# facebookresearch/holo_diffusion

Measured on AMD Instinct MI355X. Metric: denoise-steps/sec + rendered-rays/sec, 64^3x32 grid @400^2 render, higher is better.
Workload: dtype f32

## Files before the change

holo_diffusion_amd/csrc/holo_common.h:

```cpp
#pragma once

#include <stddef.h>
#include <stdint.h>
#include <stdlib.h>

#ifdef HOLO_EMU
#include "emu_runtime.h"
struct f32x2 {
  float x, y;
};
static inline f32x2 pk_fma(f32x2 a, f32x2 b, f32x2 c) { return f32x2{std::fma(a.x, b.x, c.x), std::fma(a.y, b.y, c.y)}; }
static inline f32x2 pk_mul(f32x2 a, f32x2 b) { return f32x2{a.x * b.x, a.y * b.y}; }
static inline f32x2 pk_add(f32x2 a, f32x2 b) { return f32x2{a.x + b.x, a.y + b.y}; }
static inline f32x2 pk_sub(f32x2 a, f32x2 b) { return f32x2{a.x - b.x, a.y - b.y}; }
static inline uint32_t pack_bf16x2(float lo, float hi) { return emu_bf16_bits(lo) | (emu_bf16_bits(hi) << 16); }
static inline f32x4 mfma_bf16_16x16x32(float4 a, float4 b, f32x4 c) { return emu_mfma_f32_16x16x32_bf16(a, b, c); }
static inline f32x16 mfma_bf16_32x32x16(float4 a, float4 b, f32x16 c) { return emu_mfma_f32_32x32x16_bf16(a, b, c); }
#define HOLO_LAUNDER(x) asm volatile("" : "+r"(x))
static inline float holo_rcp(float x) { return 1.0f / x; }
static inline float holo_rcp_exact(float x) { return 1.0f / x; }
static inline float holo_exp2(float x) { return std::exp2(x); }
static inline float holo_max_xor32(float x) { return std::fmax(x, __shfl_xor(x, 32)); }
static inline float holo_add_xor32(float x) { return x + __shfl_xor(x, 32); }
#define HOLO_WAVE_SYNC() emu_wave().bar.wait()
template <typename T>
static inline T holo_ld_sys(const T* p) { return *p; }
#define HOLO_PROBE_CLOCK() 0ull
#define HOLO_PROBE_HWID(hw, xcc) ((hw) = 0u, (xcc) = 0u)
#define HOLO_PHASE_DELAY(ticks) ((void)(ticks))
#define HOLO_UNIFORM(x) (x)
#define HOLO_PIN_ACC(x) ((void)0)
#define HOLO_MFMA16_ACC(acc, a, b) ((acc) = emu_mfma_f32_16x16x4f32((a), (b), (acc)))
#define HOLO_MFMA16_ACC_FIRST(acc, a, b) ((acc) = emu_mfma_f32_16x16x4f32((a), (b), (acc)))
#define HOLO_MFMA_DRAIN() ((void)0)
#define HOLO_ACC_READ(dst, acc, r) ((dst) = (acc)[r])
#define HOLO_MAD_U24(a, b, c) ((a) * (b) + (c))
#define HOLO_SINK8(a, b, c, d, e, f, g, h) ((void)0)
#define HOLO_PIN_V2(x) ((void)0)
#define HOLO_ATOMIC_ADD_F32(ptr, v) atomicAdd((ptr), (v))
#else
#include <hip/hip_runtime.h>
typedef float f32x16 __attribute__((ext_vector_type(16)));
typedef float f32x4 __attribute__((ext_vector_type(4)));
typedef float f32x2 __attribute__((ext_vector_type(2)));
__device__ __forceinline__ f32x2 pk_fma(f32x2 a, f32x2 b, f32x2 c) { return __builtin_elementwise_fma(a, b, c); }
__device__ __forceinline__ f32x2 pk_mul(f32x2 a, f32x2 b) { return a * b; }
__device__ __forceinline__ f32x2 pk_add(f32x2 a, f32x2 b) { return a + b; }
__device__ __forceinline__ f32x2 pk_sub(f32x2 a, f32x2 b) { return a - b; }
typedef __bf16 holo_bf16x2 __attribute__((ext_vector_type(2)));
typedef __bf16 holo_bf16x8 __attribute__((ext_vector_type(8)));
__device__ __forceinline__ uint32_t pack_bf16x2(float lo, float hi) {
  const holo_bf16x2 v = {(__bf16)lo, (__bf16)hi};
  return __builtin_bit_cast(uint32_t, v);
}
__device__ __forceinline__ f32x4 mfma_bf16_16x16x32(float4 a, float4 b, f32x4 c) {
  return __builtin_amdgcn_mfma_f32_16x16x32_bf16(__builtin_bit_cast(holo_bf16x8, a), __builtin_bit_cast(holo_bf16x8, b), c,
                                                 0, 0, 0);
}
__device__ __forceinline__ f32x16 mfma_bf16_32x32x16(float4 a, float4 b, f32x16 c) {
  return __builtin_amdgcn_mfma_f32_32x32x16_bf16(__builtin_bit_cast(holo_bf16x8, a), __builtin_bit_cast(holo_bf16x8, b), c,
                                                 0, 0, 0);
}
__device__ __forceinline__ float holo_rcp(float x) { return __builtin_amdgcn_rcpf(x); }
__device__ __forceinline__ float holo_exp2(float x) { return __builtin_amdgcn_exp2f(x); }
__device__ __forceinline__ float holo_max_xor32(float x) {
  const auto r = __builtin_amdgcn_permlane32_swap(__float_as_uint(x), __float_as_uint(x), false, false);
  return fmaxf(__uint_as_float(r[0]), __uint_as_float(r[1]));
}
__device__ __forceinline__ float holo_add_xor32(float x) {
  const auto r = __builtin_amdgcn_permlane32_swap(__float_as_uint(x), __float_as_uint(x), false, false);
  return __uint_as_float(r[0]) + __uint_as_float(r[1]);
}
__device__ __forceinline__ float holo_rcp_exact(float x) { return 1.0f / x; }
#define HOLO_LAUNCH(kernel, grid, block, stream, ...) \
  hipLaunchKernelGGL(kernel, grid, block, 0, (hipStream_t)(stream), __VA_ARGS__)
#define HOLO_LAUNDER(x) asm volatile("" : "+v"(x))
#define HOLO_WAVE_SYNC()                                   \
  do {                                                     \
    __builtin_amdgcn_fence(__ATOMIC_RELEASE, "wavefront"); \
    __builtin_amdgcn_wave_barrier();                       \
    __builtin_amdgcn_fence(__ATOMIC_ACQUIRE, "wavefront"); \
  } while (0)
template <typename T>
__device__ __forceinline__ T holo_ld_sys(const T* p) {
  return __hip_atomic_load(p, __ATOMIC_RELAXED, __HIP_MEMORY_SCOPE_SYSTEM);
}
#define HOLO_UNIFORM(x) __builtin_amdgcn_readfirstlane(x)
#define HOLO_PIN_ACC(x) asm volatile("" : "+a"(x))
#define HOLO_MFMA16_ACC(acc, a, b) asm volatile("v_mfma_f32_16x16x4_f32 %0, %1, %2, %0" : "+a"(acc) : "v"(a), "v"(b))
#define HOLO_MFMA16_ACC_FIRST(acc, a, b) \
  asm volatile("s_nop 1\n\tv_mfma_f32_16x16x4_f32 %0, %1, %2, %0" : "+a"(acc) : "v"(a), "v"(b))
#define HOLO_MFMA_DRAIN() asm volatile("s_nop 15" ::: "memory")
#define HOLO_ACC_READ(dst, acc, r) asm volatile("v_accvgpr_read_b32 %0, %1" : "=v"(dst) : "a"((acc)[r]))
#define HOLO_MAD_U24(a, b, c) (__umul24((a), (b)) + (c))
#define HOLO_PIN_V2(x) asm volatile("" : "+v"(x))
#define HOLO_ATOMIC_ADD_F32(ptr, v) unsafeAtomicAdd((ptr), (v))
#define HOLO_SINK8(a, b, c, d, e, f, g, h) asm volatile("" ::"v"(a), "v"(b), "v"(c), "v"(d), "v"(e), "v"(f), "v"(g), "v"(h))
#define HOLO_PROBE_CLOCK() wall_clock64()
#define HOLO_PHASE_DELAY(ticks)                                                      \
  do {                                                                               \
    unsigned hw_;                                                                    \
    asm volatile("s_getreg_b32 %0, hwreg(HW_REG_HW_ID)" : "=s"(hw_));                \
    if ((ticks) > 0 && (hw_ & 1u)) {                                                 \
      const unsigned long long t_ = wall_clock64();                                  \
      while (wall_clock64() - t_ < (unsigned long long)(ticks)) __builtin_amdgcn_s_sleep(16); \
    }                                                                                \
  } while (0)
#define HOLO_PROBE_HWID(hw, xcc)                                          \
  do {                                                                    \
    asm volatile("s_getreg_b32 %0, hwreg(HW_REG_HW_ID)" : "=s"(hw));      \
    asm volatile("s_getreg_b32 %0, hwreg(HW_REG_XCC_ID)" : "=s"(xcc));    \
  } while (0)
#endif

#define HOLO_WAVE 64

__device__ __forceinline__ float bf_lo_f32(uint32_t pk) { return __uint_as_float(pk << 16); }
__device__ __forceinline__ float bf_hi_f32(uint32_t pk) { return __uint_as_float(pk & 0xffff0000u); }
__device__ __forceinline__ void split3_pair(float x0, float x1, uint32_t& h, uint32_t& m, uint32_t& l) {
  h = pack_bf16x2(x0, x1);
  const float r0 = x0 - bf_lo_f32(h), r1 = x1 - bf_hi_f32(h);
  m = pack_bf16x2(r0, r1);
  l = pack_bf16x2(r0 - bf_lo_f32(m), r1 - bf_hi_f32(m));
}

#define HOLO_FIX_BITS 40
__device__ __forceinline__ int holo_fix_shift(uint32_t maxbits) { return HOLO_FIX_BITS - 1 - ((int)((maxbits >> 23) & 0xffu) - 127); }
__device__ __forceinline__ void holo_fix_add(long long* p, float v, int shift) {
  const long long q = (long long)rint(ldexp((double)v, shift));
  atomicAdd(reinterpret_cast<unsigned long long*>(p), (unsigned long long)q);
}
__device__ __forceinline__ float holo_fix_value(long long q, int shift) { return (float)ldexp((double)q, -shift); }

namespace holo {

void set_error(const char* fmt, ...);
const char* get_error();

static inline int64_t cdiv(int64_t a, int64_t b) { return (a + b - 1) / b; }

}
```

holo_diffusion_amd/csrc/kernels_conv3.hip:

```cpp
#include <stdio.h>
#include <stdlib.h>

#include <type_traits>
#include <utility>

#include "holo_common.h"
#include "holo_kernels.h"

#ifndef W3_PROBE
#define W3_PROBE 0
#endif
#ifndef W3_WDIST
#define W3_WDIST 3
#endif
#ifndef W3_ENTRY
#define W3_ENTRY conv_wino3_launch
#endif

namespace holo {

namespace {

constexpr int W3_BK = 32;
constexpr int W3_RS = 36;
constexpr int W3_HY = 10, W3_HX = 10;
constexpr int W3_PLANE = W3_HY * W3_HX;
constexpr int W3_HALO = 4 * W3_PLANE * W3_RS;
constexpr int W3_WSUB = 4 * 256;
constexpr int W3_WCHUNK = 32 * W3_WSUB;
constexpr int W3_WSKIP = 4 * W3_WSUB;

__device__ __forceinline__ float w3_silu(float v) { return v * holo_rcp(1.0f + __expf(-v)); }

struct w3q {
  f32x2 lo, hi;
};
__device__ __forceinline__ w3q w3_ld(const float* p) {
  const float4 v = *reinterpret_cast<const float4*>(p);
  return w3q{f32x2{v.x, v.y}, f32x2{v.z, v.w}};
}
#ifdef HOLO_EMU
struct w3_rsrc {
  const char* base;
};
static inline w3_rsrc w3_make_rsrc(const void* p) { return w3_rsrc{reinterpret_cast<const char*>(p)}; }
static inline w3q w3_bld(const w3_rsrc& r, unsigned voff, unsigned soff) {
  return w3_ld(reinterpret_cast<const float*>(r.base + (size_t)voff + (size_t)soff));
}
static inline float w3_bld1(const w3_rsrc& r, unsigned voff, unsigned soff) {
  return *reinterpret_cast<const float*>(r.base + (size_t)voff + (size_t)soff);
}
static inline void w3_bst1(const w3_rsrc& r, unsigned voff, unsigned soff, float v) {
  *reinterpret_cast<float*>(const_cast<char*>(r.base) + (size_t)voff + (size_t)soff) = v;
}
static inline void w3_bst_d2(const w3_rsrc& r, unsigned voff, unsigned soff, double a, double b) {
  double* d = reinterpret_cast<double*>(const_cast<char*>(r.base) + (size_t)voff + (size_t)soff);
  d[0] = a, d[1] = b;
}
#else
typedef __amdgpu_buffer_rsrc_t w3_rsrc;
typedef unsigned w3u4 __attribute__((ext_vector_type(4)));
__device__ __forceinline__ w3_rsrc w3_make_rsrc(const void* p) {
  return __builtin_amdgcn_make_buffer_rsrc(const_cast<void*>(p), 0, 0xffffffff, 0x00020000);
}
__device__ __forceinline__ w3q w3_bld(w3_rsrc r, unsigned voff, unsigned soff) {
  const w3u4 v = __builtin_amdgcn_raw_buffer_load_b128(r, voff, soff, 0);
  return w3q{f32x2{__uint_as_float(v.x), __uint_as_float(v.y)}, f32x2{__uint_as_float(v.z), __uint_as_float(v.w)}};
}
__device__ __forceinline__ float w3_bld1(w3_rsrc r, unsigned voff, unsigned soff) {
  return __uint_as_float(__builtin_amdgcn_raw_buffer_load_b32(r, voff, soff, 0));
}
__device__ __forceinline__ void w3_bst1(w3_rsrc r, unsigned voff, unsigned soff, float v) {
  __builtin_amdgcn_raw_buffer_store_b32(__float_as_uint(v), r, voff, soff, 0);
}
__device__ __forceinline__ void w3_bst_d2(w3_rsrc r, unsigned voff, unsigned soff, double a, double b) {
  const unsigned long long ua = __builtin_bit_cast(unsigned long long, a), ub = __builtin_bit_cast(unsigned long long, b);
  const w3u4 v = {(unsigned)ua, (unsigned)(ua >> 32), (unsigned)ub, (unsigned)(ub >> 32)};
  __builtin_amdgcn_raw_buffer_store_b128(v, r, voff, soff, 0);
}
#endif
__device__ __forceinline__ w3q w3_add(const w3q& a, const w3q& b) { return w3q{pk_add(a.lo, b.lo), pk_add(a.hi, b.hi)}; }
__device__ __forceinline__ w3q w3_sub(const w3q& a, const w3q& b) { return w3q{pk_sub(a.lo, b.lo), pk_sub(a.hi, b.hi)}; }

template <class F, int... K>
__device__ __forceinline__ void w3_static_for(F&& f, std::integer_sequence<int, K...>) {
  (f(std::integral_constant<int, K>{}), ...);
}

template <bool SKIP, bool XF>
__global__ __launch_bounds__(256, 1) void conv_wino3_kernel(ConvParams p) {
  __shared__ __attribute__((aligned(16))) float s_halo[2 * W3_HALO];

  const int tid = threadIdx.x;
  const int lane = tid & 63;
  const int wn = HOLO_UNIFORM(tid >> 6);
  const int lj = lane & 15;
  const int kq = lane >> 4;
  const int Cin = p.C0 + p.C1;
  const int ncc = (Cin + W3_BK - 1) / W3_BK;
  const int SCin = p.skip_C0 + p.skip_C1;
  const int ntx = p.OW >> 3, nty = p.OH >> 3, ntz = p.OD >> 1;
  const int ntiles = p.N * ntz * nty * ntx;
  const int ny = (p.Cout + 63) >> 6;
  const int nitems = ntiles * ny * p.nsplit;
  const int SD = p.ups ? (p.ID >> 1) : p.ID;
  const int SH = p.ups ? (p.IH >> 1) : p.IH;
  const int SW = p.ups ? (p.IW >> 1) : p.IW;
  const int wnsl = p.CoutP >> 4;
  const int64_t M = (int64_t)p.N * p.OD * p.OH * p.OW;

  struct Item {
    int n, tz0, ty0, tx0, n0, split, cc_begin, cc_end, sk_begin, sk_end;
  };
  const int X = ((W3_PROBE & 128) && (nty & 7) == 0 && (gridDim.x & 7) == 0) ? 8 : 1;
  const int ntyh = nty / X;
  const int lane_x = (int)blockIdx.x % X, G = (int)gridDim.x / X, nq = nitems / X;
  auto chunks_of = [&](Item& I) {
    I.cc_begin = I.split * p.chunks_per_split;
    I.cc_end = min(I.cc_begin + p.chunks_per_split, ncc);
    const int nsk = SKIP ? (SCin + W3_BK - 1) / W3_BK : 0;
    I.sk_begin = min(I.split * p.skip_chunks_per_split, nsk);
    I.sk_end = min(I.sk_begin + p.skip_chunks_per_split, nsk);
  };
  auto decode = [&](int qi, Item& I, int lane_ofs) {
    int t = qi;
    I.tx0 = (t % ntx) << 3;
    t /= ntx;
    I.tz0 = (t % ntz) * 2;
    t /= ntz;
    I.ty0 = ((t % ntyh) * X + lane_ofs) << 3;
    t /= ntyh;
    I.n = t % p.N;
    t /= p.N;
    I.n0 = (t % ny) * 64;
    I.split = t / ny;
    chunks_of(I);
  };
  Item stride;
  decode(G % (nq > 0 ? nq : 1), stride, 0);
  auto advance = [&](const Item& a, Item& I) {
    int tx = a.tx0 + stride.tx0, c = tx >= p.OW ? 1 : 0;
    I.tx0 = tx - (c ? p.OW : 0);
    int tz = a.tz0 + stride.tz0 + 2 * c;
    c = tz >= p.OD ? 1 : 0;
    I.tz0 = tz - (c ? p.OD : 0);
    int ty = a.ty0 + stride.ty0 + 8 * X * c;
    c = ty >= p.OH ? 1 : 0;
    I.ty0 = ty - (c ? p.OH : 0);
    int n = a.n + stride.n + c;
    c = n >= p.N ? 1 : 0;
    I.n = n - (c ? p.N : 0);
    int nb = a.n0 + stride.n0 + 64 * c;
    c = nb >= 64 * ny ? 1 : 0;
    I.n0 = nb - (c ? 64 * ny : 0);
    I.split = a.split + stride.split + c;
    chunks_of(I);
  };

  const int q = tid & 7;
  w3q hrA[4], hrB[4];
  unsigned h_off[4];
  unsigned h_cvalid = 0;
  unsigned h_zvalid = 0;
  unsigned h_zoff[4];
  const w3_rsrc rsrc0 = w3_make_rsrc(p.src0), rsrc1 = w3_make_rsrc(p.src1 ? p.src1 : p.src0);
  bool h_second = false;
  bool h_chvalid = false;
  float4 h_c01 = make_float4(1.f, 0.f, 1.f, 0.f), h_c23 = h_c01;
  auto halo_setup = [&](const Item& I, int cc) {
    int c = cc * W3_BK + q * 4;
    h_chvalid = c < Cin;
    if (!h_chvalid) c = 0;
    const bool second = p.src1 != nullptr && cc * W3_BK >= p.C0;
    const int Cs = second ? p.C1 : p.C0;
    const int cs = second ? c - p.C0 : c;
    if (XF) {
      const float4* cf = reinterpret_cast<const float4*>(p.coef + ((int64_t)I.n * Cin + c) * 2);
      h_c01 = cf[0], h_c23 = cf[1];
    }
    const unsigned cbytes = (unsigned)Cs * 4u;
    h_second = second;
    h_zvalid = 0;
#pragma unroll
    for (int pl = 0; pl < 4; ++pl) {
      int z = I.tz0 + pl - 1;
      h_zvalid |= (z >= 0 && z < p.ID ? 1u : 0u) << pl;
      z = min(max(z, 0), p.ID - 1) >> p.ups;
      h_zoff[pl] = (unsigned)((I.n * SD + z) * SH * SW) * cbytes;
    }
    h_cvalid = 0;
#pragma unroll
    for (int i = 0; i < 4; ++i) {
      const int col = min((tid >> 3) + 32 * i, W3_PLANE - 1);
      const int hy = col / W3_HX, hx = col - hy * W3_HX;
      int y = I.ty0 + hy - 1, x = I.tx0 + hx - 1;
      const bool ok = y >= 0 && y < p.IH && x >= 0 && x < p.IW;
      y = min(max(y, 0), p.IH - 1) >> p.ups;
      x = min(max(x, 0), p.IW - 1) >> p.ups;
      h_cvalid |= (ok ? 1u : 0u) << i;
      h_off[i] = (unsigned)(y * SW + x) * cbytes + (unsigned)cs * 4u;
    }
  };
  auto halo_load = [&](int i, int pl) {
    const w3q v = h_second ? w3_bld(rsrc1, h_off[i], h_zoff[pl]) : w3_bld(rsrc0, h_off[i], h_zoff[pl]);
    if (i & 1)
      hrB[pl] = v;
    else
      hrA[pl] = v;
  };
  auto commit_item_on = [&](w3q(&H)[4], int i, float* buf) {
    f32x2* V[8] = {&H[0].lo, &H[0].hi, &H[1].lo, &H[1].hi, &H[2].lo, &H[2].hi, &H[3].lo, &H[3].hi};
    if (XF && !(W3_PROBE & 64)) {
      f32x2 e[8];
      const f32x2 ca[2] = {f32x2{h_c01.x, h_c01.z}, f32x2{h_c23.x, h_c23.z}}, cb[2] = {f32x2{h_c01.y, h_c01.w}, f32x2{h_c23.y, h_c23.w}};
#pragma unroll
      for (int j = 0; j < 8; ++j) *V[j] = pk_fma(*V[j], ca[j & 1], cb[j & 1]);
      __builtin_amdgcn_sched_barrier(0);
#pragma unroll
      for (int j = 0; j < 8; ++j) e[j] = pk_mul(*V[j], f32x2{-1.4426950408889634f, -1.4426950408889634f});
      __builtin_amdgcn_sched_barrier(0);
#pragma unroll
      for (int j = 0; j < 8; ++j) e[j] = f32x2{holo_exp2(e[j].x), holo_exp2(e[j].y)};
      __builtin_amdgcn_sched_barrier(0);
#pragma unroll
      for (int j = 0; j < 8; ++j) e[j] = pk_add(e[j], f32x2{1.f, 1.f});
      __builtin_amdgcn_sched_barrier(0);
#pragma unroll
      for (int j = 0; j < 8; ++j) e[j] = f32x2{holo_rcp(e[j].x), holo_rcp(e[j].y)};
      __builtin_amdgcn_sched_barrier(0);
#pragma unroll
      for (int j = 0; j < 8; ++j) *V[j] = pk_mul(*V[j], e[j]);
      __builtin_amdgcn_sched_barrier(0);
    }
    const float kc = (h_chvalid && ((h_cvalid >> i) & 1u)) ? 1.f : 0.f;
#pragma unroll
    for (int j = 0; j < 8; ++j) {
      const float keep = ((h_zvalid >> (j >> 1)) & 1u) ? kc : 0.f;
      *V[j] = pk_mul(*V[j], f32x2{keep, keep});
    }
    const int col = min((tid >> 3) + 32 * i, W3_PLANE - 1);
    float* dst = buf + col * W3_RS + q * 4;
    const w3q o0 = w3_sub(H[0], H[2]), o1 = w3_add(H[1], H[2]), o2 = w3_sub(H[2], H[1]), o3 = w3_sub(H[1], H[3]);
    *reinterpret_cast<float4*>(dst + 0 * W3_PLANE * W3_RS) = make_float4(o0.lo.x, o0.lo.y, o0.hi.x, o0.hi.y);
    *reinterpret_cast<float4*>(dst + 1 * W3_PLANE * W3_RS) = make_float4(o1.lo.x, o1.lo.y, o1.hi.x, o1.hi.y);
    *reinterpret_cast<float4*>(dst + 2 * W3_PLANE * W3_RS) = make_float4(o2.lo.x, o2.lo.y, o2.hi.x, o2.hi.y);
    *reinterpret_cast<float4*>(dst + 3 * W3_PLANE * W3_RS) = make_float4(o3.lo.x, o3.lo.y, o3.hi.x, o3.hi.y);
  };
  auto commit_item = [&](int i, float* buf) {
    if (i & 1)
      commit_item_on(hrB, i, buf);
    else
      commit_item_on(hrA, i, buf);
  };

  f32x4 acc[64];
  const int a_off = ((2 * (lj & 3)) * W3_HX + 2 * (lj >> 2)) * W3_RS + kq * 4;
  w3q P[4][4];
  w3q Y[2][4];
  auto load_patch_row = [&](const float* buf, int step, int a) {
    const float* base = buf + a_off + ((step >> 1) * W3_PLANE + a * W3_HX) * W3_RS + (step & 1) * 16;
#pragma unroll
    for (int b = 0; b < 4; ++b) P[a][b] = w3_ld(base + b * W3_RS);
  };
  auto xform_row_half = [&](int a, int h) {
    if (h == 0) {
      const w3q t0 = w3_sub(P[a][0], P[a][2]), t3 = w3_sub(P[a][1], P[a][3]);
      P[a][0] = t0, P[a][3] = t3;
    } else {
      const w3q t1 = w3_add(P[a][1], P[a][2]), t2 = w3_sub(P[a][2], P[a][1]);
      P[a][1] = t1, P[a][2] = t2;
    }
  };
  auto yform1 = [&](int xy, int b) {
    return xy == 0 ? w3_sub(P[0][b], P[2][b]) : xy == 1 ? w3_add(P[1][b], P[2][b]) : xy == 2 ? w3_sub(P[2][b], P[1][b]) : w3_sub(P[1][b], P[3][b]);
  };
  w3q Bdummy[4] = {};
  w3q Bw[4][4];
  auto mfma1 = [&](f32x4& c, const w3q& A, const w3q& B, int e, bool first) {
#if W3_PROBE & 8
    HOLO_SINK8(A.lo.x, A.lo.y, A.hi.x, A.hi.y, B.lo.x, B.lo.y, B.hi.x, B.hi.y);
    return;
#endif
    const float a = e == 0 ? A.lo.x : e == 1 ? A.lo.y : e == 2 ? A.hi.x : A.hi.y;
    const float b = e == 0 ? B.lo.x : e == 1 ? B.lo.y : e == 2 ? B.hi.x : B.hi.y;
    if (first)
      HOLO_MFMA16_ACC_FIRST(c, a, b);
    else
      HOLO_MFMA16_ACC(c, a, b);
  };

  auto mfma16 = [&](f32x4& c0, f32x4& c1, f32x4& c2, f32x4& c3, const w3q (&A)[4], const w3q (&B)[4]) {
#pragma unroll
    for (int e = 0; e < 4; ++e) {
      mfma1(c0, A[0], B[0], e, e == 0);
      mfma1(c1, A[1], B[1], e, false);
      mfma1(c2, A[2], B[2], e, false);
      mfma1(c3, A[3], B[3], e, false);
    }
  };

  unsigned long long* dbg = p.dbg ? p.dbg + (int64_t)blockIdx.x * 8 : nullptr;
  if (dbg && tid == 0) dbg[0] = HOLO_PROBE_CLOCK();

  int it = (int)blockIdx.x / X;
  if (it >= nq) return;
  Item cur, nxt;
  decode(it, cur, lane_x);
  auto w_of = [&](const Item& I, int cc) { return (unsigned)((cc * wnsl + (I.n0 >> 4) + wn) * W3_WCHUNK) * 4u; };
  const w3_rsrc rsrcw = w3_make_rsrc(p.w_wino3);
  const unsigned lane16 = (unsigned)lane * 16u;
  auto w_ld = [&](unsigned ubase, int ofs_floats) { return w3_bld(rsrcw, lane16, ubase + (unsigned)ofs_floats * 4u); };

  int stage = 0;
  int cc = cur.cc_begin;
#pragma unroll
  for (int g = 0; g < W3_WDIST; ++g)
#pragma unroll
    for (int t = 0; t < 4; ++t) Bw[g][t] = w_ld(w_of(cur, cc), g * W3_WSUB + t * 256);
  halo_setup(cur, cc);
#pragma unroll
  for (int hp = 0; hp < 2; ++hp) {
#pragma unroll
    for (int i = 2 * hp; i < 2 * hp + 2; ++i)
#pragma unroll
      for (int pl = 0; pl < 4; ++pl) halo_load(i, pl);
#pragma unroll
    for (int i = 2 * hp; i < 2 * hp + 2; ++i) commit_item(i, s_halo);
  }
  __syncthreads();
#pragma unroll
  for (int a = 0; a < 4; ++a) load_patch_row(s_halo, 0, a);
#pragma unroll
  for (int a = 0; a < 4; ++a) {
    xform_row_half(a, 0);
    xform_row_half(a, 1);
  }
#pragma unroll
  for (int b = 0; b < 4; ++b) Y[0][b] = yform1(0, b);
  if (dbg && tid == 0) dbg[1] = HOLO_PROBE_CLOCK();

#ifdef W3_TIMELINE
  unsigned long long tl[7] = {0, 0, 0, 0, 0, 0, 0};
#endif
  for (;;) {
#pragma unroll
    for (int s = 0; s < 64; ++s)
#pragma unroll
      for (int r = 0; r < 4; ++r) acc[s][r] = 0.f;
    cc = cur.cc_begin;
    do {
      const bool last_chunk = cc + 1 == cur.cc_end;
      int ncc_ = cc + 1;
      nxt = cur;
      if (last_chunk) {
        const int nit = it + G;
        if (nit < nq) {
          advance(cur, nxt);
          ncc_ = nxt.cc_begin;
        } else {
          ncc_ = cc;
        }
      }
      const float* buf = s_halo + (stage & 1) * W3_HALO;
      float* obuf = s_halo + ((stage + 1) & 1) * W3_HALO;
      const unsigned wp = w_of(cur, cc), wnext = w_of(nxt, ncc_);
#ifdef W3_TIMELINE
      const unsigned long long t_stage = HOLO_PROBE_CLOCK();
#endif
      auto group = [&](auto gc) {
        constexpr int g = decltype(gc)::value, st = g >> 2, xy = g & 3;
#ifdef W3_TIMELINE
        const unsigned long long tA0 = clock64();
#endif
        if (g == 28) __syncthreads();
#ifdef W3_TIMELINE
        const unsigned long long tA = clock64();
        if (g == 28) tl[5] += tA - tA0;
#endif
        auto slot = [&](auto kc) {
          constexpr int k = decltype(kc)::value;
          mfma1(acc[(st >> 1) * 16 + xy * 4 + (k & 3)], Y[g & 1][k & 3], Bw[g & 3][k & 3], k >> 2, k == 0);
          if ((k & 3) == 0 && !(W3_PROBE & 2)) {
            const unsigned wsrc = g + W3_WDIST < 32 ? wp : wnext;
            constexpr int wofs = (g + W3_WDIST < 32 ? g + W3_WDIST : g + W3_WDIST - 32) * W3_WSUB + (k >> 2) * 256;
            if (W3_PROBE & 16)
              Bdummy[k >> 2] = w_ld(wsrc, wofs);
            else
              Bw[(g + W3_WDIST) & 3][k >> 2] = w_ld(wsrc, wofs);
          }
          if (xy == 3 && k < 8 && !(W3_PROBE & 4)) {
            const float* pb = st < 7 ? buf : obuf;
            constexpr int nstep = st < 7 ? st + 1 : 0;
            const float* base = pb + a_off + ((nstep >> 1) * W3_PLANE + (k >> 1) * W3_HX) * W3_RS + (nstep & 1) * 16;
            P[k >> 1][(2 * k) & 3] = w3_ld(base + ((2 * k) & 3) * W3_RS);
            P[k >> 1][(2 * k + 1) & 3] = w3_ld(base + ((2 * k + 1) & 3) * W3_RS);
          }
          if (((g >= 1 && g <= 4) || (g >= 16 && g <= 19)) && (k == 2 || k == 10) && !(W3_PROBE & 1)) {
            constexpr int hl = (g >= 16 ? g - 16 : g >= 1 ? g - 1 : 0) * 2 + (k == 10 ? 1 : 0);
            halo_load((g >= 16 ? 2 : 0) + (hl >> 2), hl & 3);
          }
          __builtin_amdgcn_sched_barrier(0);
        };
        w3_static_for(slot, std::make_integer_sequence<int, 16>{});
#ifdef W3_TIMELINE
        const unsigned long long tB = clock64();
        tl[0] += tB - tA;
#endif
        if (!(W3_PROBE & 4)) {
          if (xy == 3) {
#pragma unroll
            for (int a = 0; a < 4; ++a) {
              xform_row_half(a, 0);
              xform_row_half(a, 1);
            }
          }
#pragma unroll
          for (int b = 0; b < 4; ++b) Y[(g + 1) & 1][b] = yform1((xy + 1) & 3, b);
        }
        if (!(W3_PROBE & 1)) {
          if (g == 0) halo_setup(nxt, ncc_);
          if (!(W3_PROBE & 32)) {
            if (g == 8) commit_item(0, obuf);
            if (g == 12) commit_item(1, obuf);
            if (g == 20) commit_item(2, obuf);
            if (g == 24) commit_item(3, obuf);
          }
        }
        __builtin_amdgcn_sched_barrier(0);
#ifdef W3_TIMELINE
        tl[g == 0 ? 4 : (g == 8 || g == 12 || g == 20 || g == 24) ? 3 : xy == 3 ? 2 : 1] += clock64() - tB;
        if (g == 0) tl[6] += 1;
#endif
      };
      w3_static_for(group, std::make_integer_sequence<int, 32>{});
#ifdef W3_TIMELINE
      if (dbg && tid == 0) dbg[6] += HOLO_PROBE_CLOCK() - t_stage;
#endif
      ++stage;
    } while (++cc < cur.cc_end);
    if (SKIP) {
      const int nsg = (cur.sk_end - cur.sk_begin) * 4;
      if (nsg > 0) {
        const w3_rsrc rs0 = w3_make_rsrc(p.skip_src0), rs1 = w3_make_rsrc(p.skip_src1 ? p.skip_src1 : p.skip_src0);
        const w3_rsrc rsw = w3_make_rsrc(p.skip_w_wino3);
        const int yt = lj & 3, xt = lj >> 2;
        unsigned vrel[4];
#pragma unroll
        for (int d = 0; d < 4; ++d) vrel[d] = (unsigned)((2 * yt + (d >> 1)) * p.OW + 2 * xt + (d & 1));
        const unsigned vtile = (unsigned)(((cur.n * p.OD + cur.tz0) * p.OH + cur.ty0) * p.OW + cur.tx0);
        const unsigned zvox = (unsigned)(p.OH * p.OW);
        const unsigned wbase = (unsigned)((cur.n0 >> 4) + wn) * (unsigned)W3_WSKIP * 4u;
        auto skip_load = [&](int sg, int slot) {
          const int sc = cur.sk_begin + (sg >> 2), half = (sg >> 1) & 1, dz = sg & 1;
          const int c0 = sc * W3_BK + half * 16;
          const bool pad = c0 >= SCin;
          const bool second = !pad && c0 >= p.skip_C0;
          const unsigned Cs = (unsigned)(second ? p.skip_C1 : p.skip_C0);
          const unsigned cs = pad ? 0u : (unsigned)(second ? c0 - p.skip_C0 : c0);
          const unsigned soff = ((vtile + (unsigned)dz * zvox) * Cs + cs) * 4u;
          const unsigned wsoff = (unsigned)sc * (unsigned)wnsl * (unsigned)W3_WSKIP * 4u + wbase + (unsigned)((half * 2 + dz) * 4) * 1024u;
          const unsigned koff = (unsigned)min(kq * 4, max((int)Cs - (int)cs - 4, 0)) * 4u;
#pragma unroll
          for (int d = 0; d < 4; ++d) {
            const unsigned voff = vrel[d] * Cs * 4u + koff;
            P[slot][d] = second ? w3_bld(rs1, voff, soff) : w3_bld(rs0, voff, soff);
            Bw[slot][d] = w3_bld(rsw, lane16, wsoff + (unsigned)d * 1024u);
          }
        };
#pragma unroll
        for (int g0 = 0; g0 < 3; ++g0)
          if (g0 < nsg) skip_load(g0, g0);
        for (int sg = 0; sg < nsg; sg += 4) {
#pragma unroll
          for (int j = 0; j < 4; ++j) {
            if (sg + j + 3 < nsg) skip_load(sg + j + 3, (j + 3) & 3);
            __builtin_amdgcn_sched_barrier(0);
            if (j & 1)
              mfma16(acc[48], acc[51], acc[60], acc[63], P[j], Bw[j]);
            else
              mfma16(acc[0], acc[3], acc[12], acc[15], P[j], Bw[j]);
            __builtin_amdgcn_sched_barrier(0);
          }
        }
        const unsigned wn0 = w_of(nxt, nxt.cc_begin);
#pragma unroll
        for (int g0 = 0; g0 < W3_WDIST; ++g0)
#pragma unroll
          for (int t = 0; t < 4; ++t) Bw[g0][t] = w_ld(wn0, g0 * W3_WSUB + t * 256);
      }
    }
    if (dbg && tid == 0) dbg[2] = HOLO_PROBE_CLOCK();
    HOLO_MFMA_DRAIN();
#if W3_PROBE & 16
    HOLO_SINK8(Bdummy[0].lo, Bdummy[0].hi, Bdummy[1].lo, Bdummy[1].hi, Bdummy[2].lo, Bdummy[2].hi, Bdummy[3].lo, Bdummy[3].hi);
#endif
#if W3_PROBE & 32
    HOLO_SINK8(hrA[0].lo, hrA[1].lo, hrA[2].lo, hrA[3].lo, hrB[0].lo, hrB[1].lo, hrB[2].lo, hrB[3].lo);
#endif

    {
      const bool direct = p.nsplit == 1;
      const bool has_res = direct && p.residual != nullptr;
      int ln = lane;
      HOLO_LAUNDER(ln);
      const unsigned cout4 = (unsigned)p.Cout * 4u;
      const unsigned e_lj = (unsigned)(ln & 15) * 4u;
      const unsigned e_voff = HOLO_MAD_U24((unsigned)(ln >> 4) * 2u, cout4, e_lj);
      const unsigned cbase = (unsigned)(cur.n0 + wn * 16);
      float bv = 0.f;
      if (direct && p.bias) bv = w3_bld1(w3_make_rsrc(p.bias), e_lj, cbase * 4u);
      if (direct && p.skip_bias) bv += w3_bld1(w3_make_rsrc(p.skip_bias), e_lj, cbase * 4u);
      const unsigned vtile = (unsigned)(((cur.n * p.OD + cur.tz0) * p.OH + cur.ty0) * p.OW + cur.tx0);
      const unsigned sbase = vtile * cout4 + cbase * 4u;
      const unsigned obase = direct ? sbase : sbase + (unsigned)cur.split * ((unsigned)M * cout4);
      const unsigned zstride = (unsigned)(p.OH * p.OW) * cout4, ystride = (unsigned)p.OW * cout4;
      const w3_rsrc rs_out = w3_make_rsrc(direct ? p.out : p.partial), rs_res = w3_make_rsrc(p.residual);
      auto vofs = [&](int r, int dz, int dy, int dx) {
        return (unsigned)dz * zstride + (unsigned)(2 * r + dy) * ystride + (unsigned)dx * cout4;
      };
      float res[2][2][2][2];
      auto load_res = [&](int r) {
#pragma unroll
        for (int dz = 0; dz < 2; ++dz)
#pragma unroll
          for (int dy = 0; dy < 2; ++dy)
#pragma unroll
            for (int dx = 0; dx < 2; ++dx) res[r & 1][dz][dy][dx] = 0.f;
        if (has_res) {
#pragma unroll
          for (int dz = 0; dz < 2; ++dz)
#pragma unroll
            for (int dy = 0; dy < 2; ++dy)
#pragma unroll
              for (int dx = 0; dx < 2; ++dx) res[r & 1][dz][dy][dx] = w3_bld1(rs_res, e_voff, sbase + vofs(r, dz, dy, dx));
        }
      };
      load_res(0);
      float ssum = 0.f, ssq = 0.f;
#pragma unroll
      for (int r = 0; r < 4; ++r) {
        if (r < 3) load_res(r + 1);
        f32x2 oz[2][2][2];
#pragma unroll
        for (int zp = 0; zp < 2; ++zp) {
          f32x2 oy[4][2];
#pragma unroll
          for (int xy = 0; xy < 4; ++xy) {
            const int s0 = (2 * zp) * 16 + xy * 4, s1 = s0 + 16;
            float a0, a1, a2, a3, b0, b1, b2, b3;
            HOLO_ACC_READ(a0, acc[s0 + 0], r);
            HOLO_ACC_READ(b0, acc[s1 + 0], r);
            HOLO_ACC_READ(a1, acc[s0 + 1], r);
            HOLO_ACC_READ(b1, acc[s1 + 1], r);
            HOLO_ACC_READ(a2, acc[s0 + 2], r);
            HOLO_ACC_READ(b2, acc[s1 + 2], r);
            HOLO_ACC_READ(a3, acc[s0 + 3], r);
            HOLO_ACC_READ(b3, acc[s1 + 3], r);
            const f32x2 m0 = f32x2{a0, b0}, m1 = f32x2{a1, b1}, m2 = f32x2{a2, b2}, m3 = f32x2{a3, b3};
            oy[xy][0] = pk_add(pk_add(m0, m1), m2);
            oy[xy][1] = pk_sub(pk_sub(m1, m2), m3);
          }
#pragma unroll
          for (int dx = 0; dx < 2; ++dx) {
            oz[zp][0][dx] = pk_add(pk_add(oy[0][dx], oy[1][dx]), oy[2][dx]);
            oz[zp][1][dx] = pk_sub(pk_sub(oy[1][dx], oy[2][dx]), oy[3][dx]);
          }
          __builtin_amdgcn_sched_barrier(0);
        }
        if (SKIP && r == 3 && cur.sk_end > cur.sk_begin) {
          const float* nbuf = s_halo + (stage & 1) * W3_HALO;
#pragma unroll
          for (int a4 = 0; a4 < 4; ++a4) load_patch_row(nbuf, 0, a4);
        }
#pragma unroll
        for (int dy = 0; dy < 2; ++dy)
#pragma unroll
          for (int dx = 0; dx < 2; ++dx) {
            const f32x2 za = oz[0][dy][dx], zb = oz[1][dy][dx];
            float o0 = (za.x + za.y) + zb.x;
            float o1 = (za.y - zb.x) - zb.y;
            if (direct) {
              o0 = (o0 + res[r & 1][0][dy][dx]) + bv;
              o1 = (o1 + res[r & 1][1][dy][dx]) + bv;
              ssum += o0 + o1;
              ssq = fmaf(o0, o0, fmaf(o1, o1, ssq));
            }
            w3_bst1(rs_out, e_voff, obase + vofs(r, 0, dy, dx), o0);
            w3_bst1(rs_out, e_voff, obase + vofs(r, 1, dy, dx), o1);
          }
        __builtin_amdgcn_sched_barrier(0);
      }
      if (p.stats && direct) {
        float s1 = ssum, s2 = ssq;
        s1 += __shfl_xor(s1, 16);
        s2 += __shfl_xor(s2, 16);
        s1 += __shfl_xor(s1, 32);
        s2 += __shfl_xor(s2, 32);
        if (kq == 0) {
          const int tiles_per_sample = ntx * nty * ntz;
          const int slab = ((cur.tz0 >> 1) * nty + (cur.ty0 >> 3)) * ntx + (cur.tx0 >> 3);
          const unsigned rec = ((unsigned)(cur.n * tiles_per_sample + slab) * (unsigned)p.Cout + cbase) * 16u;
          w3_bst_d2(w3_make_rsrc(p.stats), e_lj * 4u, rec, (double)s1, (double)s2);
        }
      }
    }
    if (dbg && tid == 0) {
      const unsigned long long t_now = HOLO_PROBE_CLOCK();
      atomicAdd(dbg + 5, t_now - dbg[2]);
      dbg[3] = t_now;
      atomicAdd(dbg + 7, 1ull);
    }
    it += G;
    if (it >= nq) break;
    if (SKIP && cur.sk_end > cur.sk_begin) {
#pragma unroll
      for (int a4 = 0; a4 < 4; ++a4) {
        xform_row_half(a4, 0);
        xform_row_half(a4, 1);
      }
#pragma unroll
      for (int b4 = 0; b4 < 4; ++b4) Y[0][b4] = yform1(0, b4);
    }
    cur = nxt;
  }
#ifdef W3_TIMELINE
  if (p.dbg && tid == 0) {
    unsigned long long* d = p.dbg + ((int64_t)gridDim.x + blockIdx.x) * 8;
#pragma unroll
    for (int i = 0; i < 7; ++i) d[i] = tl[i];
  }
#endif
}

__global__ __launch_bounds__(256) void repack_conv_weight_wino3_kernel(const float* __restrict__ w, float* __restrict__ out,
                                                                       int Cout, int Cin, int src_taps, int CoutP, int CinP) {
  const int per = src_taps == 27 ? W3_WCHUNK : W3_WSKIP;
  const int nsl = CoutP >> 4;
  const int64_t total = (int64_t)(CinP >> 5) * nsl * per;
  const double G[4][3] = {{1.0, 0.0, 0.0}, {0.5, 0.5, 0.5}, {0.5, -0.5, 0.5}, {0.0, 0.0, 1.0}};
  for (int64_t i = (int64_t)blockIdx.x * blockDim.x + threadIdx.x; i < total; i += (int64_t)gridDim.x * blockDim.x) {
    const int e = (int)(i & 3);
    const int lj = (int)((i >> 2) & 15);
    const int kq = (int)((i >> 6) & 3);
    int g = (int)((i % per) >> 8);
    const int64_t blk = i / per;
    const int slice = (int)(blk % nsl);
    const int cc = (int)(blk / nsl);
    const int co = slice * 16 + lj;
    float v = 0.f;
    if (src_taps == 27) {
      const int xx = g & 3, xy = (g >> 2) & 3, half = (g >> 4) & 1, xz = g >> 5;
      const int ci = cc * 32 + half * 16 + kq * 4 + e;
      if (ci < Cin && co < Cout) {
        const float* src = w + ((int64_t)co * Cin + ci) * 27;
        double u = 0.0;
        for (int kz = 0; kz < 3; ++kz)
          for (int ky = 0; ky < 3; ++ky)
            for (int kx = 0; kx < 3; ++kx) u += G[xz][kz] * G[xy][ky] * G[xx][kx] * (double)holo_ld_sys(src + kz * 9 + ky * 3 + kx);
        v = (float)u;
      }
    } else {
      const int d = g & 3, dz = (g >> 2) & 1, half = g >> 3;
      const int ci = cc * 32 + half * 16 + kq * 4 + e;
      if (ci < Cin && co < Cout) {
        const float s = ((dz + (d >> 1) + (d & 1)) & 1) ? -1.f : 1.f;
        v = s * holo_ld_sys(w + (int64_t)co * Cin + ci);
      }
    }
    out[i] = v;
  }
}

}

#if W3_PROBE == 0 && !defined(W3_TIMELINE)
int64_t conv_wino3_weight_floats(int CoutP, int CinP, int src_taps) {
  return (int64_t)(CinP >> 5) * (CoutP >> 4) * (src_taps == 27 ? W3_WCHUNK : W3_WSKIP);
}

int repack_conv_weight_wino3_launch(const float* w, float* out, int Cout, int Cin, int src_taps, int CoutP, int CinP,
                                    void* stream) {
  const int64_t total = conv_wino3_weight_floats(CoutP, CinP, src_taps);
  int64_t blocks = (total + 255) / 256;
  if (blocks > 8192) blocks = 8192;
  HOLO_LAUNCH(repack_conv_weight_wino3_kernel, dim3((unsigned)blocks), dim3(256), stream, w, out, Cout, Cin, src_taps, CoutP,
              CinP);
  return 0;
}

#endif

int W3_ENTRY(const ConvParams& p, void* stream) {
  if (!p.w_wino3 || (p.skip_w && !p.skip_w_wino3) || (p.OD & 1) || (p.OH & 7) || (p.OW & 7) || (p.Cout & 63) ||
      (p.coef && !p.act)) {
    set_error("conv_wino3_launch: unsupported shape / weights not prepared");
    return -1;
  }
  const int ncc = (p.C0 + p.C1 + W3_BK - 1) / W3_BK;
  const int64_t out_bytes = (int64_t)p.N * p.OD * p.OH * p.OW * p.Cout * 4;
  if (p.nsplit < 1 || p.chunks_per_split < 1 || (int64_t)(p.nsplit - 1) * p.chunks_per_split >= ncc ||
      out_bytes * p.nsplit >= ((int64_t)1 << 32)) {
    set_error("conv_wino3_launch: empty K split, or output beyond 32-bit byte offsets");
    return -1;
  }
  const dim3 grid((unsigned)p.grid_x), block(256);
  if (p.skip_w && p.coef) {
    HOLO_LAUNCH((conv_wino3_kernel<true, true>), grid, block, stream, p);
  } else if (p.skip_w) {
    HOLO_LAUNCH((conv_wino3_kernel<true, false>), grid, block, stream, p);
  } else if (p.coef) {
    HOLO_LAUNCH((conv_wino3_kernel<false, true>), grid, block, stream, p);
  } else {
    HOLO_LAUNCH((conv_wino3_kernel<false, false>), grid, block, stream, p);
  }
  return 0;
}

}
```

Baseline: 162.1.

## Cut scalar/vector register pressure in wino3 conv main loop and epilogue

Removes the explicit 64x4 accumulator zeroing by issuing the first MFMA of each accumulator with a zero C operand, peeling the first stage of the chunk loop. It also hoists the per-tile halo address math out of the per-chunk setup and makes the next-item selection branchless. Epilogue parameters are reread from the kernarg segment instead of being held live in SGPRs, and the residual load uses a zero-size buffer descriptor in place of a branch. The aim is lower register pressure and fewer instructions per stage, at the cost of code-size growth from the peeled stage and reliance on ConvParams' kernarg layout.

```diff
diff --git a/holo_diffusion_amd/csrc/holo_common.h b/holo_diffusion_amd/csrc/holo_common.h
--- a/holo_diffusion_amd/csrc/holo_common.h
+++ b/holo_diffusion_amd/csrc/holo_common.h
@@ -17,6 +17,7 @@
 static inline f32x4 mfma_bf16_16x16x32(float4 a, float4 b, f32x4 c) { return emu_mfma_f32_16x16x32_bf16(a, b, c); }
 static inline f32x16 mfma_bf16_32x32x16(float4 a, float4 b, f32x16 c) { return emu_mfma_f32_32x32x16_bf16(a, b, c); }
 #define HOLO_LAUNDER(x) asm volatile("" : "+r"(x))
+#define HOLO_LAUNDER_S(x) HOLO_LAUNDER(x)
 static inline float holo_rcp(float x) { return 1.0f / x; }
 static inline float holo_rcp_exact(float x) { return 1.0f / x; }
 static inline float holo_exp2(float x) { return std::exp2(x); }
@@ -32,6 +33,8 @@
 #define HOLO_PIN_ACC(x) ((void)0)
 #define HOLO_MFMA16_ACC(acc, a, b) ((acc) = emu_mfma_f32_16x16x4f32((a), (b), (acc)))
 #define HOLO_MFMA16_ACC_FIRST(acc, a, b) ((acc) = emu_mfma_f32_16x16x4f32((a), (b), (acc)))
+#define HOLO_MFMA16_ZERO(acc, a, b) ((acc) = emu_mfma_f32_16x16x4f32((a), (b), f32x4{0.f, 0.f, 0.f, 0.f}))
+#define HOLO_MFMA16_ZERO_FIRST(acc, a, b) HOLO_MFMA16_ZERO(acc, a, b)
 #define HOLO_MFMA_DRAIN() ((void)0)
 #define HOLO_ACC_READ(dst, acc, r) ((dst) = (acc)[r])
 #define HOLO_MAD_U24(a, b, c) ((a) * (b) + (c))
@@ -75,6 +78,7 @@
 #define HOLO_LAUNCH(kernel, grid, block, stream, ...) \
   hipLaunchKernelGGL(kernel, grid, block, 0, (hipStream_t)(stream), __VA_ARGS__)
 #define HOLO_LAUNDER(x) asm volatile("" : "+v"(x))
+#define HOLO_LAUNDER_S(x) asm volatile("" : "+s"(x))
 #define HOLO_WAVE_SYNC()                                   \
   do {                                                     \
     __builtin_amdgcn_fence(__ATOMIC_RELEASE, "wavefront"); \
@@ -90,6 +94,9 @@
 #define HOLO_MFMA16_ACC(acc, a, b) asm volatile("v_mfma_f32_16x16x4_f32 %0, %1, %2, %0" : "+a"(acc) : "v"(a), "v"(b))
 #define HOLO_MFMA16_ACC_FIRST(acc, a, b) \
   asm volatile("s_nop 1\n\tv_mfma_f32_16x16x4_f32 %0, %1, %2, %0" : "+a"(acc) : "v"(a), "v"(b))
+#define HOLO_MFMA16_ZERO(acc, a, b) asm volatile("v_mfma_f32_16x16x4_f32 %0, %1, %2, 0" : "=a"(acc) : "v"(a), "v"(b))
+#define HOLO_MFMA16_ZERO_FIRST(acc, a, b) \
+  asm volatile("s_nop 1\n\tv_mfma_f32_16x16x4_f32 %0, %1, %2, 0" : "=a"(acc) : "v"(a), "v"(b))
 #define HOLO_MFMA_DRAIN() asm volatile("s_nop 15" ::: "memory")
 #define HOLO_ACC_READ(dst, acc, r) asm volatile("v_accvgpr_read_b32 %0, %1" : "=v"(dst) : "a"((acc)[r]))
 #define HOLO_MAD_U24(a, b, c) (__umul24((a), (b)) + (c))
diff --git a/holo_diffusion_amd/csrc/kernels_conv3.hip b/holo_diffusion_amd/csrc/kernels_conv3.hip
--- a/holo_diffusion_amd/csrc/kernels_conv3.hip
+++ b/holo_diffusion_amd/csrc/kernels_conv3.hip
@@ -20,6 +20,14 @@
 namespace holo {
 
 namespace {
+
+#ifdef HOLO_EMU
+#define W3_KARGS(kp) const ConvParams* kp = &p
+#else
+#define W3_KARGS(kp)                                                                                        \
+  auto kp = (const ConvParams __attribute__((address_space(4)))*)(__builtin_amdgcn_kernarg_segment_ptr()); \
+  asm volatile("" : "+s"(kp))
+#endif
 
 constexpr int W3_BK = 32;
 constexpr int W3_RS = 36;
@@ -44,10 +52,14 @@
   const char* base;
 };
 static inline w3_rsrc w3_make_rsrc(const void* p) { return w3_rsrc{reinterpret_cast<const char*>(p)}; }
+static inline w3_rsrc w3_make_rsrc_n(const void* p, unsigned nbytes) {
+  return w3_rsrc{nbytes ? reinterpret_cast<const char*>(p) : nullptr};
+}
 static inline w3q w3_bld(const w3_rsrc& r, unsigned voff, unsigned soff) {
   return w3_ld(reinterpret_cast<const float*>(r.base + (size_t)voff + (size_t)soff));
 }
 static inline float w3_bld1(const w3_rsrc& r, unsigned voff, unsigned soff) {
+  if (!r.base) return 0.f;
   return *reinterpret_cast<const float*>(r.base + (size_t)voff + (size_t)soff);
 }
 static inline void w3_bst1(const w3_rsrc& r, unsigned voff, unsigned soff, float v) {
@@ -63,6 +75,9 @@
 __device__ __forceinline__ w3_rsrc w3_make_rsrc(const void* p) {
   return __builtin_amdgcn_make_buffer_rsrc(const_cast<void*>(p), 0, 0xffffffff, 0x00020000);
 }
+__device__ __forceinline__ w3_rsrc w3_make_rsrc_n(const void* p, unsigned nbytes) {
+  return __builtin_amdgcn_make_buffer_rsrc(const_cast<void*>(p), 0, nbytes, 0x00020000);
+}
 __device__ __forceinline__ w3q w3_bld(w3_rsrc r, unsigned voff, unsigned soff) {
   const w3u4 v = __builtin_amdgcn_raw_buffer_load_b128(r, voff, soff, 0);
   return w3q{f32x2{__uint_as_float(v.x), __uint_as_float(v.y)}, f32x2{__uint_as_float(v.z), __uint_as_float(v.w)}};
@@ -87,6 +102,8 @@
   (f(std::integral_constant<int, K>{}), ...);
 }
 
+static_assert(std::is_trivially_copyable<ConvParams>::value && std::is_standard_layout<ConvParams>::value,
+              "W3_KARGS reads ConvParams straight from the kernarg segment");
 template <bool SKIP, bool XF>
 __global__ __launch_bounds__(256, 1) void conv_wino3_kernel(ConvParams p) {
   __shared__ __attribute__((aligned(16))) float s_halo[2 * W3_HALO];
@@ -167,7 +184,36 @@
   bool h_second = false;
   bool h_chvalid = false;
   float4 h_c01 = make_float4(1.f, 0.f, 1.f, 0.f), h_c23 = h_c01;
-  auto halo_setup = [&](const Item& I, int cc) {
+  unsigned h_yx = 0;
+#pragma unroll
+  for (int i = 0; i < 4; ++i) {
+    const int col = min((tid >> 3) + 32 * i, W3_PLANE - 1);
+    const int hy = col / W3_HX, hx = col - hy * W3_HX;
+    h_yx |= (unsigned)(hy | (hx << 4)) << (8 * i);
+  }
+  unsigned h_vox[4];
+  unsigned h_zvox[4];
+  auto halo_tile = [&](const Item& I) {
+    h_zvalid = 0;
+#pragma unroll
+    for (int pl = 0; pl < 4; ++pl) {
+      int z = I.tz0 + pl - 1;
+      h_zvalid |= ((unsigned)z < (unsigned)p.ID ? 1u : 0u) << pl;
+      z = min(max(z, 0), p.ID - 1) >> p.ups;
+      h_zvox[pl] = (unsigned)((I.n * SD + z) * SH * SW);
+    }
+    h_cvalid = 0;
+#pragma unroll
+    for (int i = 0; i < 4; ++i) {
+      int y = I.ty0 - 1 + (int)((h_yx >> (8 * i)) & 15u), x = I.tx0 - 1 + (int)((h_yx >> (8 * i + 4)) & 15u);
+      const unsigned ok = (unsigned)((unsigned)y < (unsigned)p.IH) & (unsigned)((unsigned)x < (unsigned)p.IW);
+      y = min(max(y, 0), p.IH - 1) >> p.ups;
+      x = min(max(x, 0), p.IW - 1) >> p.ups;
+      h_cvalid |= ok << i;
+      h_vox[i] = (unsigned)(y * SW + x);
+    }
+  };
+  auto halo_chunk = [&](const Item& I, int cc) {
     int c = cc * W3_BK + q * 4;
     h_chvalid = c < Cin;
     if (!h_chvalid) c = 0;
@@ -180,26 +226,14 @@
     }
     const unsigned cbytes = (unsigned)Cs * 4u;
     h_second = second;
-    h_zvalid = 0;
-#pragma unroll
-    for (int pl = 0; pl < 4; ++pl) {
-      int z = I.tz0 + pl - 1;
-      h_zvalid |= (z >= 0 && z < p.ID ? 1u : 0u) << pl;
-      z = min(max(z, 0), p.ID - 1) >> p.ups;
-      h_zoff[pl] = (unsigned)((I.n * SD + z) * SH * SW) * cbytes;
-    }
-    h_cvalid = 0;
-#pragma unroll
-    for (int i = 0; i < 4; ++i) {
-      const int col = min((tid >> 3) + 32 * i, W3_PLANE - 1);
-      const int hy = col / W3_HX, hx = col - hy * W3_HX;
-      int y = I.ty0 + hy - 1, x = I.tx0 + hx - 1;
-      const bool ok = y >= 0 && y < p.IH && x >= 0 && x < p.IW;
-      y = min(max(y, 0), p.IH - 1) >> p.ups;
-      x = min(max(x, 0), p.IW - 1) >> p.ups;
-      h_cvalid |= (ok ? 1u : 0u) << i;
-      h_off[i] = (unsigned)(y * SW + x) * cbytes + (unsigned)cs * 4u;
-    }
+#pragma unroll
+    for (int pl = 0; pl < 4; ++pl) h_zoff[pl] = h_zvox[pl] * cbytes;
+#pragma unroll
+    for (int i = 0; i < 4; ++i) h_off[i] = h_vox[i] * cbytes + (unsigned)cs * 4u;
+  };
+  auto halo_setup = [&](const Item& I, int cc) {
+    halo_tile(I);
+    halo_chunk(I, cc);
   };
   auto halo_load = [&](int i, int pl) {
     const w3q v = h_second ? w3_bld(rsrc1, h_off[i], h_zoff[pl]) : w3_bld(rsrc0, h_off[i], h_zoff[pl]);
@@ -276,17 +310,23 @@
   };
   w3q Bdummy[4] = {};
   w3q Bw[4][4];
-  auto mfma1 = [&](f32x4& c, const w3q& A, const w3q& B, int e, bool first) {
+  auto mfma1 = [&](f32x4& c, const w3q& A, const w3q& B, int e, bool first, bool zero = false) {
 #if W3_PROBE & 8
     HOLO_SINK8(A.lo.x, A.lo.y, A.hi.x, A.hi.y, B.lo.x, B.lo.y, B.hi.x, B.hi.y);
     return;
 #endif
     const float a = e == 0 ? A.lo.x : e == 1 ? A.lo.y : e == 2 ? A.hi.x : A.hi.y;
     const float b = e == 0 ? B.lo.x : e == 1 ? B.lo.y : e == 2 ? B.hi.x : B.hi.y;
-    if (first)
+    if (zero) {
+      if (first)
+        HOLO_MFMA16_ZERO_FIRST(c, a, b);
+      else
+        HOLO_MFMA16_ZERO(c, a, b);
+    } else if (first) {
       HOLO_MFMA16_ACC_FIRST(c, a, b);
-    else
+    } else {
       HOLO_MFMA16_ACC(c, a, b);
+    }
   };
 
   auto mfma16 = [&](f32x4& c0, f32x4& c1, f32x4& c2, f32x4& c3, const w3q (&A)[4], const w3q (&B)[4]) {
@@ -343,24 +383,24 @@
   unsigned long long tl[7] = {0, 0, 0, 0, 0, 0, 0};
 #endif
   for (;;) {
+#if W3_PROBE & 8
 #pragma unroll
     for (int s = 0; s < 64; ++s)
 #pragma unroll
       for (int r = 0; r < 4; ++r) acc[s][r] = 0.f;
+#endif
     cc = cur.cc_begin;
-    do {
+    auto stage_body = [&](auto opens_c) __attribute__((always_inline)) {
+      constexpr bool opens = decltype(opens_c)::value;
       const bool last_chunk = cc + 1 == cur.cc_end;
-      int ncc_ = cc + 1;
-      nxt = cur;
-      if (last_chunk) {
-        const int nit = it + G;
-        if (nit < nq) {
-          advance(cur, nxt);
-          ncc_ = nxt.cc_begin;
-        } else {
-          ncc_ = cc;
-        }
-      }
+      const bool go = last_chunk && it + G < nq;
+      Item adv;
+      advance(cur, adv);
+      nxt.n = go ? adv.n : cur.n, nxt.tz0 = go ? adv.tz0 : cur.tz0, nxt.ty0 = go ? adv.ty0 : cur.ty0;
+      nxt.tx0 = go ? adv.tx0 : cur.tx0, nxt.n0 = go ? adv.n0 : cur.n0, nxt.split = go ? adv.split : cur.split;
+      nxt.cc_begin = go ? adv.cc_begin : cur.cc_begin, nxt.cc_end = go ? adv.cc_end : cur.cc_end;
+      nxt.sk_begin = go ? adv.sk_begin : cur.sk_begin, nxt.sk_end = go ? adv.sk_end : cur.sk_end;
+      const int ncc_ = go ? adv.cc_begin : last_chunk ? cc : cc + 1;
       const float* buf = s_halo + (stage & 1) * W3_HALO;
       float* obuf = s_halo + ((stage + 1) & 1) * W3_HALO;
       const unsigned wp = w_of(cur, cc), wnext = w_of(nxt, ncc_);
@@ -379,7 +419,8 @@
 #endif
         auto slot = [&](auto kc) {
           constexpr int k = decltype(kc)::value;
-          mfma1(acc[(st >> 1) * 16 + xy * 4 + (k & 3)], Y[g & 1][k & 3], Bw[g & 3][k & 3], k >> 2, k == 0);
+          mfma1(acc[(st >> 1) * 16 + xy * 4 + (k & 3)], Y[g & 1][k & 3], Bw[g & 3][k & 3], k >> 2, k == 0,
+                opens && (st & 1) == 0 && (k >> 2) == 0);
           if ((k & 3) == 0 && !(W3_PROBE & 2)) {
             const unsigned wsrc = g + W3_WDIST < 32 ? wp : wnext;
             constexpr int wofs = (g + W3_WDIST < 32 ? g + W3_WDIST : g + W3_WDIST - 32) * W3_WSUB + (k >> 2) * 256;
@@ -437,26 +478,31 @@
       if (dbg && tid == 0) dbg[6] += HOLO_PROBE_CLOCK() - t_stage;
 #endif
       ++stage;
-    } while (++cc < cur.cc_end);
+    };
+    stage_body(std::true_type{});
+    int cc_end = cur.cc_end;
+    HOLO_LAUNDER_S(cc_end);
+    while (++cc < cc_end) stage_body(std::false_type{});
+    W3_KARGS(kp);
     if (SKIP) {
       const int nsg = (cur.sk_end - cur.sk_begin) * 4;
       if (nsg > 0) {
-        const w3_rsrc rs0 = w3_make_rsrc(p.skip_src0), rs1 = w3_make_rsrc(p.skip_src1 ? p.skip_src1 : p.skip_src0);
-        const w3_rsrc rsw = w3_make_rsrc(p.skip_w_wino3);
+        const w3_rsrc rs0 = w3_make_rsrc(kp->skip_src0), rs1 = w3_make_rsrc(kp->skip_src1 ? kp->skip_src1 : kp->skip_src0);
+        const w3_rsrc rsw = w3_make_rsrc(kp->skip_w_wino3);
         const int yt = lj & 3, xt = lj >> 2;
         unsigned vrel[4];
 #pragma unroll
-        for (int d = 0; d < 4; ++d) vrel[d] = (unsigned)((2 * yt + (d >> 1)) * p.OW + 2 * xt + (d & 1));
-        const unsigned vtile = (unsigned)(((cur.n * p.OD + cur.tz0) * p.OH + cur.ty0) * p.OW + cur.tx0);
-        const unsigned zvox = (unsigned)(p.OH * p.OW);
+        for (int d = 0; d < 4; ++d) vrel[d] = (unsigned)((2 * yt + (d >> 1)) * kp->OW + 2 * xt + (d & 1));
+        const unsigned vtile = (unsigned)(((cur.n * kp->OD + cur.tz0) * kp->OH + cur.ty0) * kp->OW + cur.tx0);
+        const unsigned zvox = (unsigned)(kp->OH * kp->OW);
         const unsigned wbase = (unsigned)((cur.n0 >> 4) + wn) * (unsigned)W3_WSKIP * 4u;
         auto skip_load = [&](int sg, int slot) {
           const int sc = cur.sk_begin + (sg >> 2), half = (sg >> 1) & 1, dz = sg & 1;
           const int c0 = sc * W3_BK + half * 16;
           const bool pad = c0 >= SCin;
-          const bool second = !pad && c0 >= p.skip_C0;
-          const unsigned Cs = (unsigned)(second ? p.skip_C1 : p.skip_C0);
-          const unsigned cs = pad ? 0u : (unsigned)(second ? c0 - p.skip_C0 : c0);
+          const bool second = !pad && c0 >= kp->skip_C0;
+          const unsigned Cs = (unsigned)(second ? kp->skip_C1 : kp->skip_C0);
+          const unsigned cs = pad ? 0u : (unsigned)(second ? c0 - kp->skip_C0 : c0);
           const unsigned soff = ((vtile + (unsigned)dz * zvox) * Cs + cs) * 4u;
           const unsigned wsoff = (unsigned)sc * (unsigned)wnsl * (unsigned)W3_WSKIP * 4u + wbase + (unsigned)((half * 2 + dz) * 4) * 1024u;
           const unsigned koff = (unsigned)min(kq * 4, max((int)Cs - (int)cs - 4, 0)) * 4u;
@@ -499,22 +545,23 @@
 #endif
 
     {
-      const bool direct = p.nsplit == 1;
-      const bool has_res = direct && p.residual != nullptr;
+      const bool direct = kp->nsplit == 1;
+      const bool has_res = direct && kp->residual != nullptr;
       int ln = lane;
       HOLO_LAUNDER(ln);
-      const unsigned cout4 = (unsigned)p.Cout * 4u;
+      const unsigned cout4 = (unsigned)kp->Cout * 4u;
       const unsigned e_lj = (unsigned)(ln & 15) * 4u;
       const unsigned e_voff = HOLO_MAD_U24((unsigned)(ln >> 4) * 2u, cout4, e_lj);
       const unsigned cbase = (unsigned)(cur.n0 + wn * 16);
       float bv = 0.f;
-      if (direct && p.bias) bv = w3_bld1(w3_make_rsrc(p.bias), e_lj, cbase * 4u);
-      if (direct && p.skip_bias) bv += w3_bld1(w3_make_rsrc(p.skip_bias), e_lj, cbase * 4u);
-      const unsigned vtile = (unsigned)(((cur.n * p.OD + cur.tz0) * p.OH + cur.ty0) * p.OW + cur.tx0);
+      if (direct && kp->bias) bv = w3_bld1(w3_make_rsrc(kp->bias), e_lj, cbase * 4u);
+      if (direct && kp->skip_bias) bv += w3_bld1(w3_make_rsrc(kp->skip_bias), e_lj, cbase * 4u);
+      const unsigned vtile = (unsigned)(((cur.n * kp->OD + cur.tz0) * kp->OH + cur.ty0) * kp->OW + cur.tx0);
       const unsigned sbase = vtile * cout4 + cbase * 4u;
       const unsigned obase = direct ? sbase : sbase + (unsigned)cur.split * ((unsigned)M * cout4);
-      const unsigned zstride = (unsigned)(p.OH * p.OW) * cout4, ystride = (unsigned)p.OW * cout4;
-      const w3_rsrc rs_out = w3_make_rsrc(direct ? p.out : p.partial), rs_res = w3_make_rsrc(p.residual);
+      const unsigned zstride = (unsigned)(kp->OH * kp->OW) * cout4, ystride = (unsigned)kp->OW * cout4;
+      const w3_rsrc rs_out = w3_make_rsrc(direct ? kp->out : kp->partial);
+      const w3_rsrc rs_res = w3_make_rsrc_n(kp->residual, HOLO_UNIFORM(has_res ? 0xffffffffu : 0u));
       auto vofs = [&](int r, int dz, int dy, int dx) {
         return (unsigned)dz * zstride + (unsigned)(2 * r + dy) * ystride + (unsigned)dx * cout4;
       };
@@ -525,15 +572,7 @@
 #pragma unroll
           for (int dy = 0; dy < 2; ++dy)
 #pragma unroll
-            for (int dx = 0; dx < 2; ++dx) res[r & 1][dz][dy][dx] = 0.f;
-        if (has_res) {
-#pragma unroll
-          for (int dz = 0; dz < 2; ++dz)
-#pragma unroll
-            for (int dy = 0; dy < 2; ++dy)
-#pragma unroll
-              for (int dx = 0; dx < 2; ++dx) res[r & 1][dz][dy][dx] = w3_bld1(rs_res, e_voff, sbase + vofs(r, dz, dy, dx));
-        }
+            for (int dx = 0; dx < 2; ++dx) res[r & 1][dz][dy][dx] = w3_bld1(rs_res, e_voff, sbase + vofs(r, dz, dy, dx));
       };
       load_res(0);
       float ssum = 0.f, ssq = 0.f;
@@ -590,7 +629,7 @@
           }
         __builtin_amdgcn_sched_barrier(0);
       }
-      if (p.stats && direct) {
+      if (kp->stats && direct) {
         float s1 = ssum, s2 = ssq;
         s1 += __shfl_xor(s1, 16);
         s2 += __shfl_xor(s2, 16);
@@ -599,8 +638,8 @@
         if (kq == 0) {
           const int tiles_per_sample = ntx * nty * ntz;
           const int slab = ((cur.tz0 >> 1) * nty + (cur.ty0 >> 3)) * ntx + (cur.tx0 >> 3);
-          const unsigned rec = ((unsigned)(cur.n * tiles_per_sample + slab) * (unsigned)p.Cout + cbase) * 16u;
-          w3_bst_d2(w3_make_rsrc(p.stats), e_lj * 4u, rec, (double)s1, (double)s2);
+          const unsigned rec = ((unsigned)(cur.n * tiles_per_sample + slab) * (unsigned)kp->Cout + cbase) * 16u;
+          w3_bst_d2(w3_make_rsrc(kp->stats), e_lj * 4u, rec, (double)s1, (double)s2);
         }
       }
     }
```

After: 165.5 (median of 6 runs). +2.1%, better.
